# brontoguana/krasis

Measured on AMD Instinct MI355X. Metric: decode tok/s, Qwen3-Coder-Next Q4 @1 MI355X (KR_DECODE_FAST tolerance mode; both modes: value_exact / value_fast), higher is better.
Workload: dtype int4-g128 w x int16 act -> i32, f32 scales; 1 GPU; Qwen3-Coder-Next Q4 int4gpu on 1×MI355X (512-expert top-10, hybrid linear+GQA, FP8 KV); kv=FP8-E4M3 KV cache, kv_max_seq 256, layers=48, parallelism=one GPU holds the whole model (N > 1 lines: expert parallelism, see main_multi), hip_graph=True

## Files before the change

### krasis_amd/csrc/kr_decode.cpp

```cpp
#include <algorithm>
#include <hip/hip_runtime.h>

#include <cmath>
#include <cstring>
#include <memory>
#include <string>
#include <vector>

#include "../../include/krasis_hip.h"
#include "kr_decode_ops.h"
#include "kr_engine_internal.h"
#include "kr_kernels.h"
#include "kr_prefill.h"
#include "kr_router.h"
#include "kr_sampler.h"
#include <chrono>

#include "kr_decode_internal.h"
#include "kr_decode_fast.h"

static void prof_mark(kr_decode_store* s, int kind, hipStream_t st) {
    if (!s->prof) return;
    if (s->ev_used + 2 > s->ev_pool.size()) { for (int i = 0; i < 64; i++) { hipEvent_t e; (void)hipEventCreate(&e); s->ev_pool.push_back(e); } }
    if (kind >= 0) s->ev_kind.push_back(kind);
// ... 273 lines not shown
    for (auto& L : s->layers) if (L.mlp == MLP_MOE && L.moe_layer >= (int)eng->layers.size())
        return kr_fail(KR_ERR_VALUE, "moe_layer_idx %d out of range (engine has %zu MoE layers)", L.moe_layer, eng->layers.size());
    kr_engine_destroy(s->eng);
    s->eng = eng; s->own_eng = false; s->graph_ok = false; s->last_stream = nullptr;
    return KR_OK;
}

extern "C" int kr_decode_set_layer_moe(kr_decode_store* s, int layer, int moe_layer_idx, int shared_gate_up_wid, int shared_down_wid, int shared_gate_wid) {
    if (int rc = need_cfg(s)) return rc;
    if (layer < 0 || layer >= (int)s->layers.size()) return kr_fail(KR_ERR_VALUE, "layer %d out of range", layer);
    if (moe_layer_idx < 0 || (!s->own_eng && moe_layer_idx >= (int)s->eng->layers.size())) return kr_fail(KR_ERR_VALUE, "moe_layer_idx %d out of range", moe_layer_idx);
    if ((shared_gate_up_wid >= 0) != (shared_down_wid >= 0)) return kr_fail(KR_ERR_VALUE, "shared gate_up and down weights must be set together");
    for (int id : {shared_gate_up_wid, shared_down_wid, shared_gate_wid}) if (id >= 0) if (int rc = chk_wid(s, id, "set_decode_layer_moe")) return rc;
    DLayer& L = s->layers[layer];
    L.mlp = MLP_MOE; L.moe_layer = moe_layer_idx; L.sgu_wid = shared_gate_up_wid; L.sd_wid = shared_down_wid; L.sg_wid = shared_gate_wid;
    s->graph_ok = false;
    return KR_OK;
}

extern "C" int kr_decode_set_layer_dense(kr_decode_store* s, int layer, int gate_wid, int up_wid, int down_wid) {
    if (int rc = need_cfg(s)) return rc;
    if (layer < 0 || layer >= (int)s->layers.size()) return kr_fail(KR_ERR_VALUE, "layer %d out of range", layer);
    for (int id : {gate_wid, up_wid, down_wid}) if (int rc = chk_wid(s, id, "set_decode_layer_dense")) return rc;
    DLayer& L = s->layers[layer];
    L.mlp = MLP_DENSE; L.gate_wid = gate_wid; L.up_wid = up_wid; L.down_wid = down_wid;
    s->graph_ok = false;
    return KR_OK;
}

extern "C" int kr_decode_set_rope(kr_decode_store* s, const float* cos_t, const float* sin_t, int half_dim, int max_seq) {
    if (int rc = need_cfg(s)) return rc;
    KR_HIP(hipSetDevice(s->eng->device));
    if (int rc = upload_f32(s->rope_cos, cos_t, (size_t)half_dim * max_seq)) return rc;
    if (int rc = upload_f32(s->rope_sin, sin_t, (size_t)half_dim * max_seq)) return rc;
    s->rope_half = half_dim; s->max_rope_seq = max_seq; s->graph_ok = false;
    return KR_OK;
}

static size_t maxz(size_t a, size_t b) { return a > b ? a : b; }

extern "C" int kr_decode_finalize(kr_decode_store* s) {
    if (int rc = need_cfg(s)) return rc;
    if ((int)s->layers.size() != s->n_layers) return kr_fail(KR_ERR_STATE, "configured %d layers but %zu were added", s->n_layers, s->layers.size());
    KR_HIP(hipSetDevice(s->eng->device));
    size_t pa = 0, pb = 0, qb = 0, kb = 0, vb = 0, zb = 0, ro = 0, ao = 0, gb = 0, dg = 0, lb = 0, fq = 64;
    for (auto& L : s->layers) {
        if (L.attn == ATTN_LA) {
            pa = maxz(pa, s->weights[L.qkvz_wid]->rows); pb = maxz(pb, s->weights[L.ba_wid]->rows);
            qb = maxz(qb, (size_t)L.nv * L.dk); kb = maxz(kb, (size_t)L.nv * L.dk); vb = maxz(vb, (size_t)L.nv * L.dv); zb = maxz(zb, (size_t)L.nv * L.dv);
            ro = maxz(ro, (size_t)L.nv * L.dv); ao = maxz(ao, s->weights[L.out_wid]->cols); gb = maxz(gb, L.nv); fq = maxz(fq, (size_t)L.nk * 2 * L.dk);
        } else if (L.attn == ATTN_GQA) {
            pa = maxz(pa, s->weights[L.q_wid]->rows); kb = maxz(kb, s->weights[L.k_wid]->rows); vb = maxz(vb, s->weights[L.v_wid]->rows);
            qb = maxz(qb, (size_t)L.nh * L.hd); zb = maxz(zb, (size_t)L.nh * L.hd); ao = maxz(ao, s->weights[L.o_wid]->cols);
        }
        else if (L.attn == ATTN_MLA) {
            const size_t hd = (size_t)L.nd + L.rd;
            pa = maxz(pa, (size_t)L.nh * hd); kb = maxz(kb, (size_t)L.klr + L.rd); qb = maxz(qb, (size_t)L.nh * L.klr); zb = maxz(zb, (size_t)L.nh * L.rd);
            lb = maxz(lb, (size_t)L.nh * L.klr); ao = maxz(ao, maxz((size_t)L.nh * L.vhd, s->weights[L.o_wid]->cols));
            if (L.mq_wid < 0) pb = maxz(pb, maxz(s->weights[L.mqa_wid]->rows, s->weights[L.mqb_wid]->cols));
        }
        if (L.mlp == MLP_DENSE) dg = maxz(dg, 2 * (size_t)s->weights[L.down_wid]->cols);
    }
    ao = maxz(ao, (size_t)s->hidden);
    {
        const size_t kh = ((size_t)s->hidden + 127) / 128 * 128, ka = (ao + 127) / 128 * 128;
        if (s->img_in.ensure(kr_act_image_bytes((int)kh)) || s->img_post.ensure(kr_act_image_bytes((int)kh)) || s->img_post_bf16.ensure(kr_act_image_bytes((int)kh)) ||
            s->img_attn.ensure(kr_act_image_bytes((int)ka)))
            return kr_fail(KR_ERR_HIP, "hipMalloc of the activation images failed");
// ... 242 lines not shown
        a.q = (float*)s->f_qk.p;
        if (PROF_RC(PK_LA_RECUR, kr_launch_la_step_heads(a, (float*)L.recur_state.p, (const float*)L.la_norm_w.p, (float*)s->attn_out.p, s->eps, st, la_img)))
            return kr_fail(KR_ERR_VALUE, "unsupported linear-attention geometry");
    } else if (la_fused) {
        (void)PROF_RC(PK_LA_RECUR, kr_launch_la_step(a, (float*)L.recur_state.p, (const float*)L.la_norm_w.p, (float*)s->attn_out.p, s->eps, st, la_img));
    } else {
        PROF(PK_LA_CONV, kr_launch_la_conv(a, st));
        if (PROF_RC(PK_LA_RECUR, kr_launch_la_recurrent_gnorm((float*)L.recur_state.p, a.q, a.k, a.v, a.g, a.beta, a.z, (const float*)L.la_norm_w.p,
                                                             (float*)s->attn_out.p, L.nv, L.dk, L.dv, s->eps, st, la_img)))
            return kr_fail(KR_ERR_VALUE, "unsupported linear-attention geometry");
    }
    out_proj(cx, L.out_wid, o_img);
    return KR_OK;
}

static int attn_gqa(StepCtx& cx, DLayer& L, size_t li) {
    kr_decode_store* s = cx.s; hipStream_t st = cx.st;
    if (!L.kv_k.p) return kr_fail(KR_ERR_STATE, "set_decode_state was not called (no KV cache for layer %zu)", li);
    if (!cx.did_in) {
        const int wids[3] = {L.q_wid, L.k_wid, L.v_wid};
        float* ys[3] = {(float*)s->proj_a.p, (float*)s->kbuf.p, (float*)s->vbuf.p};
        proj_group(cx, wids, ys, 3, cx.in_img ? (const void*)s->img_in.p : (const void*)cx.hid, cx.in_img ? 2 : 1);
    }
    KrGqaArgs a{};
    a.step = (const KrStep*)s->step_dev.p; a.q_in = (const float*)s->proj_a.p; a.k_in = (const float*)s->kbuf.p; a.v_in = (const float*)s->vbuf.p;
    a.q_norm = L.q_norm_len ? (const float*)L.q_norm.p : nullptr; a.k_norm = L.k_norm_len ? (const float*)L.k_norm.p : nullptr;
    a.q_norm_per_head = L.q_norm_len == L.nh * L.hd; a.k_norm_per_head = L.k_norm_len == L.nkv * L.hd;
    a.rope_cos = (const float*)s->rope_cos.p; a.rope_sin = (const float*)s->rope_sin.p; a.rope_half = s->rope_half;
    a.k_cache = L.kv_k.p; a.v_cache = L.kv_v.p; a.kv_fp8 = s->kv_fp8; a.q_out = (float*)s->qbuf.p; a.gate = (float*)s->gatebuf.p;
    a.attn_out = (float*)s->attn_out.p; a.gated = L.gated; a.nh = L.nh; a.nkv = L.nkv; a.hd = L.hd; a.eps = s->eps; a.sm_scale = L.sm_scale;
    const bool o_img = cx.img_ok() && img_w(s, L.o_wid) && L.hd % 128 == 0 && s->weights[L.o_wid]->cols == L.nh * L.hd;
    a.img_out = o_img ? s->img_attn.p : nullptr;
    a.sc_g = s->kv_max_seq > s->gqa_split_min ? (float*)s->gqa_scores.p : nullptr;
    a.force_stream = s->opt_gqa_stream; a.tree_norm = cx.fast ? 1 : 0;
    if (s->attn_fast && a.sc_g) { a.fd_o = (float*)s->fd_o.p; a.fd_ml = (float*)s->fd_ml.p; }
    PROF(PK_GQA, { if (!(cx.fast && s->opt_gqa_fused && !a.sc_g && kr_launch_fgqa(a, s->kv_max_seq, st) == 0)) kr_launch_gqa(a, s->kv_max_seq, st); });
    out_proj(cx, L.o_wid, o_img);
    return KR_OK;
}

static void mla_lora_tail(StepCtx& cx, DLayer& L, float* q_full) {
    kr_decode_store* s = cx.s; hipStream_t st = cx.st;
    if (L.q_a_norm_len) PROF(PK_RMSNORM, kr_launch_rmsnorm_seq((float*)s->proj_b.p, (const float*)L.q_a_norm.p, s->weights[L.mqa_wid]->rows, s->eps, st));
    PROF(PK_MATVEC, kr_launch_matvec(mv(s, L.mqb_wid), s->proj_b.p, 1, q_full, st));
}

static int attn_mla(StepCtx& cx, DLayer& L, size_t li) {
    kr_decode_store* s = cx.s; hipStream_t st = cx.st;
    if (!L.kv_k.p) return kr_fail(KR_ERR_STATE, "set_decode_state was not called (no MLA cache for layer %zu)", li);
    if (L.mla_rope_seq < s->kv_max_seq) return kr_fail(KR_ERR_VALUE, "MLA rope table (%d) shorter than kv_max_seq (%d)", L.mla_rope_seq, s->kv_max_seq);
    float* kv_out = (float*)s->kbuf.p; float* q_full = (float*)s->proj_a.p;
    const bool lora = L.mq_wid < 0;
    if (!cx.did_in) {
        const int wids[2] = {L.kva_wid, lora ? L.mqa_wid : L.mq_wid};
        float* ys[2] = {kv_out, lora ? (float*)s->proj_b.p : q_full};
        proj_group(cx, wids, ys, 2, cx.hid, 1);
    }
    if (lora) mla_lora_tail(cx, L, q_full);
    KrMlaArgs a{};
    a.step = (const KrStep*)s->step_dev.p; a.kv_out = kv_out; a.q_full = q_full; a.kv_a_norm = (const float*)L.kv_a_norm.p; a.w_kc = (const float*)L.w_kc.p;
    a.w_vc = (const float*)L.w_vc.p; a.rope_cos = (const float*)L.mla_cos.p; a.rope_sin = (const float*)L.mla_sin.p;
    a.ckv_cache = L.kv_k.p; a.kpe_cache = L.kv_v.p; a.kv_fp8 = s->kv_fp8; a.q_abs = (float*)s->qbuf.p; a.q_pe = (float*)s->zbuf.p;
    a.attn_lat = (float*)s->latbuf.p; a.v_proj = (float*)s->attn_out.p;
    a.nh = L.nh; a.klr = L.klr; a.nd = L.nd; a.rd = L.rd; a.vhd = L.vhd; a.eps = s->eps; a.sm_scale = L.sm_scale;
    a.sc_g = s->kv_max_seq > s->mla_split_min ? (float*)s->gqa_scores.p : nullptr;
    if (s->attn_fast && a.sc_g) { a.fast = 1; a.fd_o = (float*)s->fd_o.p; a.fd_ml = (float*)s->fd_ml.p; }
    a.decode_fast = cx.fast ? 1 : 0; a.decode_fused = cx.fast && s->opt_gqa_fused ? 1 : 0;
// ... 264 lines not shown
        return KR_OK;
    }
    return enqueue_step(s, st);
}

extern "C" int kr_decode_set_kv_dtype(kr_decode_store* s, int kv_dtype) {
    if (int rc = chk_store(s)) return rc;
    if (kv_dtype != 0 && kv_dtype != 1) return kr_fail(KR_ERR_VALUE, "kv_dtype %d unknown (0 = FP16, 1 = FP8-E4M3)", kv_dtype);
    if (s->kv_fp8 != kv_dtype) for (auto& L : s->layers) if (L.attn == ATTN_GQA || L.attn == ATTN_MLA) { L.kv_k.release(); L.kv_v.release(); }
    s->kv_fp8 = kv_dtype; s->graph_ok = false;
    return KR_OK;
}

extern "C" int kr_decode_set_attention_mode(kr_decode_store* s, int mode) {
    if (int rc = chk_store(s)) return rc;
    if (mode < 0 || mode > 7) return kr_fail(KR_ERR_VALUE, "numerics mode %d unknown (bit 0 = KR_ATTN_FAST, bit 1 = KR_GEMM_FAST, bit 2 = KR_DECODE_FAST)", mode);
    s->attn_fast = mode & 1; s->gemm_fast = (mode >> 1) & 1; s->decode_fast = (mode >> 2) & 1; s->graph_ok = false;
    return KR_OK;
}

extern "C" int kr_decode_set_option(kr_decode_store* s, const char* name, int value) {
    if (int rc = chk_store(s)) return rc;
    if (!name) return kr_fail(KR_ERR_VALUE, "null option name");
    if (!strcmp(name, "gqa_stream")) { s->opt_gqa_stream = value != 0; s->graph_ok = false; return KR_OK; }
    if (!strcmp(name, "w2_combine")) { s->opt_w2_combine = value != 0; s->graph_ok = false; return KR_OK; }
    if (!strcmp(name, "la_heads")) { s->opt_la_heads = value != 0; s->graph_ok = false; return KR_OK; }
    if (!strcmp(name, "lm_fused")) { s->opt_lm_fused = value != 0; s->graph_ok = false; return KR_OK; }
    if (!strcmp(name, "gqa_fused")) { s->opt_gqa_fused = value != 0; s->graph_ok = false; return KR_OK; }
    if (!strcmp(name, "gemm_ring")) { kr_pfr_set_enabled(value); return KR_OK; }
    if (!strcmp(name, "la_conv_fused")) { s->opt_la_conv_fused = value != 0; return KR_OK; }
    if (!strcmp(name, "dense_fast")) { s->opt_dense_fast = value != 0; s->graph_ok = false; return KR_OK; }
    if (!strcmp(name, "slot_select")) { s->opt_slot_select = value != 0; s->graph_ok = false; return KR_OK; }
    if (!strcmp(name, "slot_rows_late_first")) { s->opt_slot_rows_late_first = value != 0; s->graph_ok = false; return KR_OK; }
    if (!strcmp(name, "norm_rows")) { s->opt_norm_rows = value != 0; return KR_OK; }
    if (!strcmp(name, "pfm_timing")) { s->opt_pfm_timing = value != 0; return KR_OK; }
    if (!strcmp(name, "generate_lookahead")) { s->opt_gen_lookahead = value != 0; return KR_OK; }
    if (!strcmp(name, "multi_sample_loop")) { s->opt_multi_sample_loop = value != 0; return KR_OK; }
    if (!strcmp(name, "multi_attn_fast")) { s->opt_multi_attn_fast = value != 0; return KR_OK; }
    if (!strcmp(name, "multi_attn_fast_paged")) { s->opt_multi_attn_fast_paged = value != 0; return KR_OK; }
    if (!strcmp(name, "multi_mla_fast")) { s->opt_multi_mla_fast = value != 0; return KR_OK; }
    if (!strcmp(name, "multi_extend_la_chunk")) { s->opt_multi_extend_la_chunk = value != 0; return KR_OK; }
    if (!strcmp(name, "multi_extend_exact_mfma")) { s->opt_multi_extend_exact_mfma = value != 0; return KR_OK; }
    if (!strcmp(name, "multi_extend_mla_exact_mfma")) { s->opt_multi_extend_mla_exact_mfma = value != 0; return KR_OK; }
    if (!strcmp(name, "multi_attn_exact_split")) { s->opt_multi_attn_exact_split = value != 0; return KR_OK; }
    if (!strcmp(name, "multi_attn_exact_split_min")) {
        if (value < 1) return kr_fail(KR_ERR_VALUE, "multi_attn_exact_split_min %d: at least 1", value);
        s->opt_multi_attn_exact_split_min = value; return KR_OK;
    }
    if (!strcmp(name, "multi_mla_exact_split")) { s->opt_multi_mla_exact_split = value != 0; return KR_OK; }
    if (!strcmp(name, "multi_extend_la_exact")) { s->opt_multi_extend_la_exact = value != 0; return KR_OK; }
    if (!strcmp(name, "multi_extend_la_exact_min")) {
        if (value < 2 || value > 1024) return kr_fail(KR_ERR_VALUE, "multi_extend_la_exact_min %d: must be in [2, 1024]", value);
        s->opt_multi_extend_la_exact_min = value; return KR_OK;
    }
    if (!strcmp(name, "multi_mla_exact_split_min")) {
        if (value < 1) return kr_fail(KR_ERR_VALUE, "multi_mla_exact_split_min %d: at least 1", value);
        s->opt_multi_mla_exact_split_min = value; return KR_OK;
    }
    if (!strcmp(name, "multi_extend_flash")) { s->opt_multi_extend_flash = value != 0; return KR_OK; }
    if (!strcmp(name, "multi_extend_mla_flash")) { s->opt_multi_extend_mla_flash = value != 0; return KR_OK; }
    if (!strcmp(name, "gguf_exact_pass")) { s->opt_gguf_exact_pass = value != 0; return KR_OK; }
    if (!strcmp(name, "gguf_exact_grouped")) { s->opt_gguf_exact_grouped = value != 0; return KR_OK; }
    if (!strcmp(name, "pass_few_rows")) { s->opt_pass_few_rows = value != 0; return KR_OK; }
    if (!strcmp(name, "pass_few_rows_max")) {
        if (value < 1 || value > 16) return kr_fail(KR_ERR_VALUE, "pass_few_rows_max %d: 1 .. 16", value);
        s->opt_pass_few_rows_max = value; return KR_OK;
// ... 238 lines not shown
```

### krasis_amd/csrc/kr_decode_fast.hip

```cpp
#include "kr_decode_fast.h"
#include "kr_gguf_dev.h"

#include "kr_device.h"
#include "kr_libm.h"
#include "kr_exact_dev.h"
#include "kr_matvec_dev.h"
#include "kr_topk.h"

typedef float f32x4 __attribute__((ext_vector_type(4)));
extern __shared__ __attribute__((aligned(16))) u32x4 kr_fsm[];

#ifdef KR_FTIMING
__device__ unsigned long long kr_fstamps[8][16];
#define KR_FSTAMP(k, i) do { if (blockIdx.x == gridDim.x / 2 && blockIdx.y == 0 && threadIdx.x == 0) kr_fstamps[k][i] = wall_clock64(); } while (0)
#define KR_FSTAMPY(k, i, row_) do { if (blockIdx.x == gridDim.x / 2 && (int)blockIdx.y == (row_) && threadIdx.x == 0) kr_fstamps[k][i] = wall_clock64(); } while (0)
extern "C" int kr_debug_fstamps(unsigned long long* out) { return (int)hipMemcpyFromSymbol(out, HIP_SYMBOL(kr_fstamps), sizeof(kr_fstamps)); }
__device__ unsigned long long kr_fwg[6][1024][3];
#define KR_FWG(k, i) do { if (threadIdx.x == 0) { const unsigned b_ = blockIdx.x + gridDim.x * blockIdx.y; if (b_ < 1024) { kr_fwg[k][b_][i] = wall_clock64(); \
        if ((i) == 0) kr_fwg[k][b_][2] = (unsigned long long)__builtin_amdgcn_s_getreg((4 << 0) | (0 << 6) | (31 << 11)) | ((unsigned long long)__builtin_amdgcn_s_getreg((20 << 0) | (0 << 6) | (3 << 11)) << 32); } } } while (0)
extern "C" int kr_debug_fwg(unsigned long long* out) { return (int)hipMemcpyFromSymbol(out, HIP_SYMBOL(kr_fwg), sizeof(kr_fwg)); }
#else
#define KR_FSTAMP(k, i) do { } while (0)
#define KR_FSTAMPY(k, i, y) do { } while (0)
#define KR_FWG(k, i) do { } while (0)
#endif

#define KR_FW2_LDS_MAX (64 * 1024)
#define KR_FU 16

__device__ __forceinline__ float kr_f_red8(float v) {
    v += __int_as_float(KR_DPP(__float_as_int(v), KR_DPP_XOR1));
    v += __int_as_float(KR_DPP(__float_as_int(v), KR_DPP_XOR2));
    v += __int_as_float(KR_DPP(__float_as_int(v), KR_DPP_HALF_MIRROR));
    return v;
}
__device__ __forceinline__ float kr_f_red16(float v) {
    v = kr_f_red8(v);
    v += __int_as_float(KR_DPP(__float_as_int(v), KR_DPP_MIRROR));
    return v;
}
__device__ __forceinline__ float kr_f_rl(float v, int l) { return __int_as_float(__builtin_amdgcn_readlane(__float_as_int(v), l)); }
__device__ __forceinline__ float kr_f_wave_sum(float v) {
    v = kr_f_red16(v);
    return (kr_f_rl(v, 0) + kr_f_rl(v, 16)) + (kr_f_rl(v, 32) + kr_f_rl(v, 48));
}
__device__ __forceinline__ float kr_f_wave_max(float v) {
    v = kr_red16_max_f32(v);
    return fmaxf(fmaxf(kr_f_rl(v, 0), kr_f_rl(v, 16)), fmaxf(kr_f_rl(v, 32), kr_f_rl(v, 48)));
}
__device__ __forceinline__ void kr_f_wave_sync() { __builtin_amdgcn_fence(__ATOMIC_ACQ_REL, "workgroup"); __builtin_amdgcn_wave_barrier(); }

template <int BITS, int NU, int FU = KR_FU> struct KrFw { u32x4 w[NU > 0 ? NU : FU]; uint32_t sc[NU > 0 ? NU : FU]; };

template <int BITS, int NU, int FU = KR_FU>
__device__ __forceinline__ void kr_f_fetch(KrFw<BITS, NU, FU>& p, const KrMatDev& m, const void* qbase, const uint32_t* sbase, int tile, int lane, int ub, int u1) {
    const int units = BITS == 4 ? m.ngp : m.ng;
    const u32x4* q = reinterpret_cast<const u32x4*>(qbase) + (size_t)tile * units * 64 + lane;
// ... 921 lines not shown

#define KR_FGQA_MAX 1024
template <int N, bool FP8> struct KrKvRaw { static constexpr int W = FP8 ? (N + 3) / 4 : (N + 1) / 2; uint32_t w[W]; };
template <int N, bool FP8>
__device__ __forceinline__ void kr_kv_raw_load(KrKvRaw<N, FP8>& r, const void* base, size_t elem) {
    constexpr int bytes = FP8 ? N : 2 * N;
    const char* p = reinterpret_cast<const char*>(base) + elem * (FP8 ? 1 : 2);
    if constexpr (bytes >= 16) {
#pragma unroll
        for (int i = 0; i < bytes / 16; i++) { const u32x4 v = *reinterpret_cast<const u32x4*>(p + 16 * i); r.w[4 * i] = v.x; r.w[4 * i + 1] = v.y; r.w[4 * i + 2] = v.z; r.w[4 * i + 3] = v.w; }
    } else if constexpr (bytes == 8) { const u32x2 v = *reinterpret_cast<const u32x2*>(p); r.w[0] = v.x; r.w[1] = v.y; }
    else if constexpr (bytes == 4) r.w[0] = *reinterpret_cast<const uint32_t*>(p);
    else if constexpr (bytes == 2) r.w[0] = *reinterpret_cast<const uint16_t*>(p);
    else r.w[0] = *reinterpret_cast<const uint8_t*>(p);
}
template <int N, bool FP8>
__device__ __forceinline__ void kr_kv_raw_f32(const KrKvRaw<N, FP8>& r, float (&x)[N]) {
#pragma unroll
    for (int i = 0; i < N; i++) {
        if constexpr (FP8) {
            const int w = (int)r.w[i >> 2];
            x[i] = (i & 3) == 0 ? __builtin_amdgcn_cvt_f32_fp8(w, 0) : ((i & 3) == 1 ? __builtin_amdgcn_cvt_f32_fp8(w, 1) : ((i & 3) == 2 ? __builtin_amdgcn_cvt_f32_fp8(w, 2) : __builtin_amdgcn_cvt_f32_fp8(w, 3)));
        } else {
            const uint16_t hb = (uint16_t)((i & 1) ? (r.w[i >> 1] >> 16) : (r.w[i >> 1] & 0xFFFFu));
            x[i] = (float)__builtin_bit_cast(_Float16, hb);
        }
    }
}
template <bool FP8> __device__ __forceinline__ float kr_kv_round(float v) {
    if constexpr (FP8) return kr_e4m3_to_f32(kr_f32_to_e4m3(v));
    else return (float)(_Float16)v;
}

template <int HD, bool FP8>
__global__ void __launch_bounds__(256) kr_fgqa_kernel(const KrStep* p_step, const float* p_q, const float* p_k, const float* p_v, const void* p_kc, const void* p_vc,
                                                      int p_nh, int p_nkv, const KrGqaArgs a) {
    constexpr int D16 = HD / 16;
    constexpr int DPL = HD / 64;
    constexpr int SB = 2;
    constexpr int PB = 8;
    __shared__ __attribute__((aligned(16))) float s_q[HD], s_k[HD], s_v[HD], s_sc[KR_FGQA_MAX + 64], s_part[4][HD];
    __shared__ float s_red[2][4];
    const int h = blockIdx.x, t = threadIdx.x, wave = t >> 6, lane = t & 63;
    const int grp = p_nh / p_nkv, kvh = h / grp;
    const int pos = p_step->pos, seq = pos + 1;
    const size_t rowe = (size_t)p_nkv * HD, headoff = (size_t)kvh * HD;
    const int d = t < HD ? t : HD - 1;
    const bool own = t < HD;
    const float qraw = a.gated ? p_q[(size_t)h * HD * 2 + d] : p_q[(size_t)h * HD + d];
    const float graw = a.gated ? p_q[(size_t)h * HD * 2 + HD + d] : 0.0f;
    const float kraw = p_k[headoff + d], vraw = p_v[headoff + d];
    const float qw = a.q_norm ? a.q_norm[(a.q_norm_per_head ? h * HD : 0) + d] : 1.0f;
    const float kw = a.k_norm ? a.k_norm[(a.k_norm_per_head ? kvh * HD : 0) + d] : 1.0f;
    const int d2 = a.rope_half;
    const bool rot = t < 2 * d2 && own;
    const int ri = rot ? (t < d2 ? t : t - d2) : 0;
    const float rc = a.rope_cos[(size_t)pos * d2 + ri], rs = a.rope_sin[(size_t)pos * d2 + ri];
    const int l16 = lane & 15, pw = lane >> 4;
    KrKvRaw<D16, FP8> kqA[SB], kqB[SB];
    auto issue_k = [&](KrKvRaw<D16, FP8> (&kq)[SB], int s0) {
#pragma unroll
        for (int u = 0; u < SB; u++) { const int sp = s0 + 16 * u + wave * 4 + pw; kr_kv_raw_load<D16, FP8>(kq[u], p_kc, (size_t)(sp < pos ? sp : 0) * rowe + headoff + l16 * D16); }
    };
    issue_k(kqA, 0);
    float sq = own ? qraw * qraw : 0.0f, sk = own ? kraw * kraw : 0.0f;
    sq = kr_f_wave_sum(sq); sk = kr_f_wave_sum(sk);
    if (lane == 0) { s_red[0][wave] = sq; s_red[1][wave] = sk; }
    __syncthreads();
    float qx = qraw, kx = kraw;
    if (a.q_norm) { const float ss = (s_red[0][0] + s_red[0][1]) + (s_red[0][2] + s_red[0][3]); qx = qraw * (kr_rms_inv(ss, HD, a.eps) * qw); }
    if (a.k_norm) { const float ss = (s_red[1][0] + s_red[1][1]) + (s_red[1][2] + s_red[1][3]); kx = kraw * (kr_rms_inv(ss, HD, a.eps) * kw); }
    if (own) { s_q[t] = qx; s_k[t] = kx; }
    __syncthreads();
    float qv = qx, kv = kx;
    if (rot) {
        if (t < d2) { qv = qx * rc - s_q[d2 + t] * rs; kv = kx * rc - s_k[d2 + t] * rs; }
        else { qv = qx * rc + s_q[t - d2] * rs; kv = kx * rc + s_k[t - d2] * rs; }
    }
    __syncthreads();
    if (own) {
        s_q[t] = qv; s_k[t] = kr_kv_round<FP8>(kv); s_v[t] = kr_kv_round<FP8>(vraw);
        if (h == kvh * grp) {
            const size_t o = (size_t)pos * rowe + headoff + t;
            kr_kv_store(const_cast<void*>(p_kc), o, kv, FP8 ? 1 : 0);
            kr_kv_store(const_cast<void*>(p_vc), o, vraw, FP8 ? 1 : 0);
        }
    }
    __syncthreads();
    float qreg[D16], knew[D16];
#pragma unroll
    for (int i = 0; i < D16; i++) { qreg[i] = s_q[l16 * D16 + i]; knew[i] = s_k[l16 * D16 + i]; }
    auto score_batch = [&](const KrKvRaw<D16, FP8> (&kq)[SB], int s0) {
#pragma unroll
        for (int u = 0; u < SB; u++) {
            const int sp = s0 + 16 * u + wave * 4 + pw;
            float kx_[D16];
            kr_kv_raw_f32<D16, FP8>(kq[u], kx_);
            float acc = 0.0f;
#pragma unroll
            for (int i = 0; i < D16; i++) acc = __builtin_fmaf(qreg[i], sp == pos ? knew[i] : kx_[i], acc);
            acc = kr_f_red16(acc);
            if (l16 == 0 && sp < seq) s_sc[sp] = acc * a.sm_scale;
        }
    };
    constexpr int SSTEP = 16 * SB;
    for (int s0 = 0; s0 < seq; s0 += 2 * SSTEP) {
        if (s0 + SSTEP < seq) issue_k(kqB, s0 + SSTEP);
        score_batch(kqA, s0);
        if (s0 + 2 * SSTEP < seq) issue_k(kqA, s0 + 2 * SSTEP);
        if (s0 + SSTEP < seq) score_batch(kqB, s0 + SSTEP);
    }
    KrKvRaw<DPL, FP8> vqA[PB], vqB[PB];
    auto issue_v = [&](KrKvRaw<DPL, FP8> (&vq)[PB], int s0) {
#pragma unroll
        for (int u = 0; u < PB; u++) { const int sp = s0 + 4 * u + wave; kr_kv_raw_load<DPL, FP8>(vq[u], p_vc, (size_t)(sp < pos ? sp : 0) * rowe + headoff + lane * DPL); }
    };
    issue_v(vqA, 0);
    __syncthreads();
    float mx = -__builtin_inff();
    for (int sp = t; sp < seq; sp += 256) mx = fmaxf(mx, s_sc[sp]);
    mx = kr_f_wave_max(mx);
    if (lane == 0) s_red[0][wave] = mx;
    __syncthreads();
    mx = fmaxf(fmaxf(s_red[0][0], s_red[0][1]), fmaxf(s_red[0][2], s_red[0][3]));
    float se = 0.0f;
    for (int sp = t; sp < seq; sp += 256) { const float e = kr_expf(s_sc[sp] - mx); s_sc[sp] = e; se += e; }
    se = kr_f_wave_sum(se);
    if (lane == 0) s_red[1][wave] = se;
    __syncthreads();
    const float inv = 1.0f / ((s_red[1][0] + s_red[1][1]) + (s_red[1][2] + s_red[1][3]));
    for (int sp = t; sp < seq; sp += 256) s_sc[sp] *= inv;
    float vnew[DPL];
#pragma unroll
    for (int i = 0; i < DPL; i++) vnew[i] = s_v[lane * DPL + i];
    __syncthreads();
    float o[DPL];
#pragma unroll
    for (int i = 0; i < DPL; i++) o[i] = 0.0f;
    auto pv_batch = [&](const KrKvRaw<DPL, FP8> (&vq)[PB], int s0) {
#pragma unroll
        for (int u = 0; u < PB; u++) {
            const int sp = s0 + 4 * u + wave;
            float vx[DPL];
            kr_kv_raw_f32<DPL, FP8>(vq[u], vx);
            const float pr = sp < seq ? s_sc[sp] : 0.0f;
#pragma unroll
            for (int i = 0; i < DPL; i++) o[i] = __builtin_fmaf(pr, sp == pos ? vnew[i] : vx[i], o[i]);
        }
    };
    constexpr int PSTEP = 4 * PB;
    for (int s0 = 0; s0 < seq; s0 += 2 * PSTEP) {
        if (s0 + PSTEP < seq) issue_v(vqB, s0 + PSTEP);
        pv_batch(vqA, s0);
        if (s0 + 2 * PSTEP < seq) issue_v(vqA, s0 + 2 * PSTEP);
        if (s0 + PSTEP < seq) pv_batch(vqB, s0 + PSTEP);
    }
#pragma unroll
    for (int i = 0; i < DPL; i++) s_part[wave][lane * DPL + i] = o[i];
    __syncthreads();
    float ov = 0.0f;
    if (own) {
        ov = (s_part[0][t] + s_part[1][t]) + (s_part[2][t] + s_part[3][t]);
        if (a.gated) ov *= 1.0f / (1.0f + kr_expf(-graw));
        a.attn_out[(size_t)h * HD + t] = ov;
        s_q[t] = ov;
    }
    if (a.img_out) {
        __syncthreads();
        const KrActLds Lg = kr_carve_lds(reinterpret_cast<u32x4*>(a.img_out), p_nh * HD, false);
        constexpr int nch = HD / 8;
        if (t < nch) {
            float v8[8];
            kr_load8(s_q, t, v8);
            float mxq = 0.0f;
#pragma unroll
            for (int i = 0; i < 8; i++) mxq = fmaxf(mxq, fabsf(v8[i]));
            float scale, invq;
            kr_group_scale(mxq, scale, invq);
            int q8[8];
            kr_quant8<false>(v8, invq, q8);
            const int gc = h * nch + t;
            kr_store_chunk<false>(Lg, gc, q8);
            if ((gc & 15) == 0) Lg.ascale[gc >> 4] = scale;
        }
    }
}

template <int KLR, int RD, bool FP8>
__global__ void __launch_bounds__(256) kr_fmla_kernel(const KrStep* p_step, const float* p_qabs, const float* p_qpe, const void* p_ckv, const void* p_kpe, float* p_out, float p_scale) {
    constexpr int DC = KLR / 16, DR = RD / 16, DPL = KLR / 64, SB = 2, PB = 8;
    __shared__ __attribute__((aligned(16))) float s_sc[KR_FGQA_MAX + 64], s_part[4][KLR];
    __shared__ float s_red[2][4];
    const int h = blockIdx.x, t = threadIdx.x, wave = t >> 6, lane = t & 63, l16 = lane & 15, pw = lane >> 4;
    const int pos = p_step->pos, seq = pos + 1;
    KrKvRaw<DC, FP8> kcA[SB], kcB[SB]; KrKvRaw<DR, FP8> krA[SB], krB[SB];
    auto issue_k = [&](KrKvRaw<DC, FP8> (&kc)[SB], KrKvRaw<DR, FP8> (&kr)[SB], int s0) {
#pragma unroll
        for (int u = 0; u < SB; u++) {
            const int sp = s0 + 16 * u + wave * 4 + pw, sr = sp < seq ? sp : 0;
            kr_kv_raw_load<DC, FP8>(kc[u], p_ckv, (size_t)sr * KLR + l16 * DC);
            kr_kv_raw_load<DR, FP8>(kr[u], p_kpe, (size_t)sr * RD + l16 * DR);
        }
    };
    float qc[DC], qr[DR];
#pragma unroll
    for (int i = 0; i < DC; i += 4) { const float4 v = *reinterpret_cast<const float4*>(p_qabs + (size_t)h * KLR + l16 * DC + i); qc[i] = v.x; qc[i + 1] = v.y; qc[i + 2] = v.z; qc[i + 3] = v.w; }
#pragma unroll
    for (int i = 0; i < DR; i += 4) { const float4 v = *reinterpret_cast<const float4*>(p_qpe + (size_t)h * RD + l16 * DR + i); qr[i] = v.x; qr[i + 1] = v.y; qr[i + 2] = v.z; qr[i + 3] = v.w; }
    issue_k(kcA, krA, 0);
    auto score_batch = [&](const KrKvRaw<DC, FP8> (&kc)[SB], const KrKvRaw<DR, FP8> (&kr)[SB], int s0) {
#pragma unroll
        for (int u = 0; u < SB; u++) {
            const int sp = s0 + 16 * u + wave * 4 + pw;
            float xc[DC], xr[DR];
            kr_kv_raw_f32<DC, FP8>(kc[u], xc); kr_kv_raw_f32<DR, FP8>(kr[u], xr);
            float acc = 0.0f, acr = 0.0f;
#pragma unroll
            for (int i = 0; i < DC; i++) acc = __builtin_fmaf(qc[i], xc[i], acc);
// ... 39 lines not shown
        for (int u = 0; u < PB; u++) {
            const int sp = s0 + 4 * u + wave;
            float vx[DPL];
            kr_kv_raw_f32<DPL, FP8>(vq[u], vx);
            const float pr = sp < seq ? s_sc[sp] : 0.0f;
#pragma unroll
            for (int i = 0; i < DPL; i++) o[i] = __builtin_fmaf(pr, vx[i], o[i]);
        }
    };
    constexpr int PSTEP = 4 * PB;
    for (int s0 = 0; s0 < seq; s0 += 2 * PSTEP) {
        if (s0 + PSTEP < seq) issue_v(vqB, s0 + PSTEP);
        pv_batch(vqA, s0);
        if (s0 + 2 * PSTEP < seq) issue_v(vqA, s0 + 2 * PSTEP);
        if (s0 + PSTEP < seq) pv_batch(vqB, s0 + PSTEP);
    }
#pragma unroll
    for (int i = 0; i < DPL; i++) s_part[wave][lane * DPL + i] = o[i];
    __syncthreads();
    for (int j = t; j < KLR; j += 256) p_out[(size_t)h * KLR + j] = (s_part[0][j] + s_part[1][j]) + (s_part[2][j] + s_part[3][j]);
}

int kr_launch_fmla(const KrMlaArgs& a, int max_seq, hipStream_t st) {
    if (!a.step || max_seq > KR_FGQA_MAX || a.sc_g || a.rd != 64 || (a.klr != 512 && a.klr != 256)) return 1;
#define KR_FMLA(K_, F_) hipLaunchKernelGGL((kr_fmla_kernel<K_, 64, F_>), dim3(a.nh), dim3(256), 0, st, a.step, (const float*)a.q_abs, (const float*)a.q_pe, (const void*)a.ckv_cache, (const void*)a.kpe_cache, a.attn_lat, a.sm_scale)
    if (a.klr == 512) { if (a.kv_fp8) KR_FMLA(512, true); else KR_FMLA(512, false); }
    else { if (a.kv_fp8) KR_FMLA(256, true); else KR_FMLA(256, false); }
#undef KR_FMLA
    return 0;
}

int kr_launch_fgqa(const KrGqaArgs& a, int max_seq, hipStream_t st) {
    if (max_seq > KR_FGQA_MAX || a.sc_g || a.nh % a.nkv || 2 * a.rope_half > a.hd || (a.img_out && a.hd % 128)) return 1;
#define KR_FGQA(H_, F_) hipLaunchKernelGGL((kr_fgqa_kernel<H_, F_>), dim3(a.nh), dim3(256), 0, st, a.step, a.q_in, a.k_in, a.v_in, (const void*)a.k_cache, (const void*)a.v_cache, a.nh, a.nkv, a)
    if (a.hd == 256) { if (a.kv_fp8) KR_FGQA(256, true); else KR_FGQA(256, false); }
    else if (a.hd == 128) { if (a.kv_fp8) KR_FGQA(128, true); else KR_FGQA(128, false); }
    else if (a.hd == 64) { if (a.kv_fp8) KR_FGQA(64, true); else KR_FGQA(64, false); }
    else return 1;
#undef KR_FGQA
    return 0;
}

template <int BITS, int KS, int MODE>
static int kr_fdm_launch_nu2(const KrFdmArgs& a, int nu, dim3 grid, size_t lds, hipStream_t st) {
    const void* p0 = MODE == 0 ? a.img : ((MODE == 1 && a.emb) ? nullptr : (const void*)a.hid_in);
    const float* p1 = (MODE == 1 && !a.first) ? a.res_in : nullptr;
    const int Kp = a.mm.m[0].ng * 128;
#define KR_FDM(N_) hipLaunchKernelGGL((kr_fdm_kernel<BITS, KS, N_, MODE>), grid, dim3(256), lds, st, p0, p1, a.norm_w, Kp, a)
    switch (nu) {
        case 2: KR_FDM(2); break;
        case 4: KR_FDM(4); break;
        case 8: KR_FDM(8); break;
        case 16: KR_FDM(16); break;
        default: KR_FDM(0); break;
    }
#undef KR_FDM
    return 0;
}
template <int BITS, int KS>
static int kr_fdm_launch_nu(const KrFdmArgs& a, int nu, dim3 grid, size_t lds, hipStream_t st) {
    if (a.mode == 0) return kr_fdm_launch_nu2<BITS, KS, 0>(a, nu, grid, lds, st);
    if (a.mode == 2) return kr_fdm_launch_nu2<BITS, KS, 2>(a, nu, grid, lds, st);
    return kr_fdm_launch_nu2<BITS, KS, 1>(a, nu, grid, lds, st);
}

int kr_launch_fdm(const KrFdmArgs& a, hipStream_t st) {
    const KrMatDev& m0 = a.mm.m[0];
    const int bits = m0.bits, K = m0.ng * 128;
    for (int i = 1; i < a.mm.n; i++) if (a.mm.m[i].bits != bits || a.mm.m[i].ng != m0.ng) return 1;
    if ((a.mode == 1 || a.mode == 2) && (K > 4096 || K != m0.K)) return 1;
    if (a.conv_state && (a.conv_mi < 0 || a.conv_mi >= a.mm.n || a.mm.m[a.conv_mi].N != a.nk * (2 * a.dk + 2 * a.hr * a.dv) || a.gate_mi < 0 || a.gate_mi >= a.mm.n ||
                         a.mm.m[a.gate_mi].N != a.nk * 2 * a.hr || !a.ge_out || !a.beta_out)) return 1;
// ... 132 lines not shown
```

### krasis_amd/csrc/kr_decode_internal.h

```cpp
#pragma once
#include <hip/hip_runtime.h>

#include <memory>
#include <vector>

#include "kr_decode_ops.h"
#include "kr_engine_internal.h"
#include "kr_multi.h"
#include "kr_page_pool.h"
#include "kr_spec.h"

struct DWeight { MatSet ms; int rows = 0, cols = 0; };

enum { ATTN_NONE = 0, ATTN_LA = 1, ATTN_GQA = 2, ATTN_MLA = 3 };
enum { MLP_NONE = 0, MLP_MOE = 1, MLP_DENSE = 2 };

struct DLayer {
    int input_norm = -1, post_norm = -1;
    int attn = ATTN_NONE, mlp = MLP_NONE;
    int qkvz_wid = -1, ba_wid = -1, out_wid = -1, nk = 0, nv = 0, dk = 0, dv = 0, kd = 4; float la_scale = 1.0f;
    DevBuf conv_w, a_log, dt_bias, la_norm_w, conv_state, recur_state;
    int q_wid = -1, k_wid = -1, v_wid = -1, o_wid = -1, gated = 0, nh = 0, nkv = 0, hd = 0; float sm_scale = 1.0f;
    DevBuf q_norm, k_norm, kv_k, kv_v; int q_norm_len = 0, k_norm_len = 0;
    int kva_wid = -1, mq_wid = -1, mqa_wid = -1, mqb_wid = -1, klr = 0, nd = 0, rd = 0, vhd = 0, q_a_norm_len = 0;
// ... 16 lines not shown
    DevBuf lc_scratch;
    DevBuf xm_rows;
    bool mla_fd_ready = false;
    struct Sampler { float temperature = 0.0f, top_p = 1.0f, penalty = 0.0f; int top_k = 0; };
    std::vector<Sampler> smp; size_t smp_words = 0;
    DevBuf smp_seen, smp_rng;
    DevBuf smp_rows, smp_work, smp_sorted, smp_keys, smp_temp, smp_probs; size_t smp_temp_bytes = 0;
    DevBuf smp_hyp;
    DevBuf v_rec, v_tab, v_out, v_keep; std::vector<KrMultiLaCommit> v_host; std::vector<int> v_la_of;
    bool v_pending = false, v_sampled = false, v_has64 = false, v_has128 = false; int v_nv_max = 0, v_dv_max = 0; size_t v_rows = 0;
    std::vector<int32_t> v_match; hipStream_t v_st = nullptr;
    hipEvent_t ev = nullptr;
    DevBuf sw_stage, sw_pools, sw_pieces; void* sw_pinned = nullptr; size_t sw_half = 0; hipStream_t sw_stream = nullptr; hipEvent_t sw_ev[4] = {nullptr, nullptr, nullptr, nullptr};
    ~kr_multi_state() {
        if (ev) (void)hipEventDestroy(ev);
        for (hipEvent_t e : sw_ev) if (e) (void)hipEventDestroy(e);
        if (sw_stream) (void)hipStreamDestroy(sw_stream);
        if (sw_pinned) (void)hipHostFree(sw_pinned);
    }
};

struct kr_standalone_state;
struct kr_decode_store {
    kr_standalone_state* standalone = nullptr;
    kr_engine* eng = nullptr; int device = 0; bool own_eng = false;
    int group_size = 128; bool norm_bias_one = false;
    std::vector<std::unique_ptr<DWeight>> weights;
    std::vector<std::unique_ptr<DevBuf>> norms; std::vector<int> norm_len;
    bool configured = false;
    int hidden = 0, n_layers = 0, vocab = 0, topk = 0, scoring = 1, norm_topk = 1, final_norm = -1, lm_head = -1;
    float eps = 1e-6f, rsf = 1.0f;
    DevBuf embedding;
    std::vector<DLayer> layers;
    DevBuf rope_cos, rope_sin; int rope_half = 0, max_rope_seq = 0;
    int kv_max_seq = 0;
    DevBuf hid, res, proj_a, proj_b, qbuf, kbuf, vbuf, zbuf, gbuf, betabuf, gatebuf, latbuf, recur_out, attn_out, logits, gate_val, tok;
    DevBuf dense_gu;
    DevBuf hid2, res2, r_counter, argmax_scratch;
    int kv_fp8 = 0;
    DevBuf img_in, img_post, img_post_bf16, img_attn;
    int opt_gqa_stream = 0, opt_pfm_timing = 0, opt_norm_rows = 1, opt_la_conv_fused = 1, opt_gqa_fused = 1, opt_lm_fused = 1, opt_la_heads = 1, opt_w2_combine = 1, opt_dense_fast = 1, opt_slot_select = 1, opt_slot_rows_late_first = 1;
    int opt_multi_sample_loop = 0;
    int opt_gguf_exact_pass = 0;
    int opt_gguf_exact_grouped = 1;
    int opt_multi_attn_fast_paged = 0;
    int opt_multi_attn_fast = 0;
    int opt_multi_mla_fast = 0;
    int opt_multi_extend_flash = 0;
    int opt_multi_extend_la_chunk = 0;
    int opt_multi_attn_exact_split = 0;
    int opt_multi_attn_exact_split_min = 512;
    int opt_multi_extend_la_exact = 0;
    int opt_multi_extend_la_exact_min = 8;
    int opt_multi_mla_exact_split = 0;
    int opt_multi_mla_exact_split_min = 512;
    int opt_multi_extend_exact_mfma = 0;
    int opt_multi_extend_mla_exact_mfma = 0;
    int opt_multi_extend_mla_flash = 0;
    int opt_pass_few_rows = 0;
    int opt_pass_few_rows_max = 16;
    int opt_pass_few_rows_group = 0;
    int opt_slot_swap_chunk_bytes = KR_SLOT_CHUNK_DEFAULT;
    int64_t path_counts[KR_MPC_COUNT] = {};
    int opt_gen_lookahead = 0;
    int opt_ep_graph = 0;
    uint64_t ep_generation_seen = 0;
    int ep_eager_steps = 0;
    int* gen_ring = nullptr; int gen_ring_n = 0; hipEvent_t gen_ev[2] = {nullptr, nullptr};
    int decode_fast = 0; DevBuf f_qk;
    int gemm_fast = 0;
    int attn_fast = 0; DevBuf fd_o, fd_ml;
    DevBuf gqa_scores; int gqa_split_min = 1024, mla_split_min = 512;
    DevBuf smp_seen, smp_keys, smp_temp, smp_probs, smp_rng; size_t smp_temp_bytes = 0;
    DevBuf pf_scores;
// ... 36 lines not shown
```

### krasis_amd/csrc/kr_decode_ops.h

```cpp
#pragma once
#include <hip/hip_runtime.h>
#include <stdint.h>

struct KrStep { int token; int pos; };

struct KrLaArgs {
    const float* qkvz; const float* ba; float* conv_state; const float* conv_w; const float* a_log; const float* dt_bias;
    float scale; float *q, *k, *v, *z, *g, *beta; int nk, nv, dk, dv, hr;
};
struct KrGqaArgs {
    const KrStep* step;
    const float *q_in, *k_in, *v_in;
    const float *q_norm, *k_norm; int q_norm_per_head, k_norm_per_head;
    const float *rope_cos, *rope_sin; int rope_half;
    void *k_cache, *v_cache; int kv_fp8;
    float *q_out, *gate, *attn_out;
    int gated, nh, nkv, hd; float eps, sm_scale;
    void* img_out;
    float* sc_g;
    float *fd_o, *fd_ml;
    int tree_norm;
    int force_stream;
};

struct KrFdFlashArgs {
    const KrStep* step; const float* q;
    const void *k_cache, *v_cache;
    float *fd_o, *fd_ml;
    int nh, nkv; float sm_scale;
    const float* gate; int gated; float* out; void* img_out;
};
int kr_fd_flash_chunk(int max_seq);
size_t kr_fd_flash_chunks(int max_seq);
int kr_fd_flash_prepare(int hd, int fp8);
int kr_launch_fd_flash(const KrFdFlashArgs& a, int hd, int fp8, int max_seq, hipStream_t st);
int kr_gqa_attn_prepare(int max_seq, int hd, int fp8);

struct KrMlaArgs {
    const KrStep* step;
    const float* kv_out;
    const float* q_full;
    const float *kv_a_norm, *w_kc, *w_vc, *rope_cos, *rope_sin;
    void *ckv_cache, *kpe_cache;
    int kv_fp8;
    float* sc_g;
    float *fd_o, *fd_ml; int fast;
    float *q_abs, *q_pe, *attn_lat, *v_proj;
    int nh, klr, nd, rd, vhd; float eps, sm_scale;
    int pos0; int ld_kv, ld_q;
    int decode_fast;
    int decode_fused;
    int absorb_done;
    float* pf_sc; int pf_sc_ld;
};
void kr_launch_mla(const KrMlaArgs& a, int max_seq, hipStream_t s, int n_tok = 1);
// ... 27 lines not shown
```

Before: 642.5 tok/s.

## Prefetch a window of KV cache rows before norm/rope in fused GQA decode kernel

Adds a templated prefetch path to the fused GQA decode kernel. It issues K loads for the first 128 positions into registers and V rows into registers (later staged into LDS) at kernel start, before the q/k norm and rope work. The aim is to hide the KV cache memory latency behind that prologue instead of serialising it. The path is on by default through a new attn_prefetch option, and in exchange it raises register and shared memory pressure, which may reduce occupancy. Timing stamps are also extended for KR_FTIMING builds.

```diff
diff --git a/krasis_amd/csrc/kr_decode.cpp b/krasis_amd/csrc/kr_decode.cpp
--- a/krasis_amd/csrc/kr_decode.cpp
+++ b/krasis_amd/csrc/kr_decode.cpp
@@ -329,8 +329,7 @@
     if (int rc = need_cfg(s)) return rc;
     KR_HIP(hipSetDevice(s->eng->device));
     if (int rc = upload_f32(s->rope_cos, cos_t, (size_t)half_dim * max_seq)) return rc;
-    if (int rc = upload_f32(s->rope_sin, sin_t, (size_t)half_dim * max_seq)) return rc;
-    s->rope_half = half_dim; s->max_rope_seq = max_seq; s->graph_ok = false;
+    if (int rc = upload_f32(s->rope_sin, sin_t, (size_t)half_dim * max_seq)) return rc;    s->rope_half = half_dim; s->max_rope_seq = max_seq; s->graph_ok = false;
     return KR_OK;
 }
 
@@ -639,7 +638,7 @@
     const bool o_img = cx.img_ok() && img_w(s, L.o_wid) && L.hd % 128 == 0 && s->weights[L.o_wid]->cols == L.nh * L.hd;
     a.img_out = o_img ? s->img_attn.p : nullptr;
     a.sc_g = s->kv_max_seq > s->gqa_split_min ? (float*)s->gqa_scores.p : nullptr;
-    a.force_stream = s->opt_gqa_stream; a.tree_norm = cx.fast ? 1 : 0;
+    a.force_stream = s->opt_gqa_stream; a.tree_norm = cx.fast ? 1 : 0; a.attn_prefetch = s->opt_attn_prefetch;
     if (s->attn_fast && a.sc_g) { a.fd_o = (float*)s->fd_o.p; a.fd_ml = (float*)s->fd_ml.p; }
     PROF(PK_GQA, { if (!(cx.fast && s->opt_gqa_fused && !a.sc_g && kr_launch_fgqa(a, s->kv_max_seq, st) == 0)) kr_launch_gqa(a, s->kv_max_seq, st); });
     out_proj(cx, L.o_wid, o_img);
@@ -970,6 +969,7 @@
     if (!strcmp(name, "dense_fast")) { s->opt_dense_fast = value != 0; s->graph_ok = false; return KR_OK; }
     if (!strcmp(name, "slot_select")) { s->opt_slot_select = value != 0; s->graph_ok = false; return KR_OK; }
     if (!strcmp(name, "slot_rows_late_first")) { s->opt_slot_rows_late_first = value != 0; s->graph_ok = false; return KR_OK; }
+    if (!strcmp(name, "attn_prefetch")) { s->opt_attn_prefetch = value != 0; s->graph_ok = false; return KR_OK; }
     if (!strcmp(name, "norm_rows")) { s->opt_norm_rows = value != 0; return KR_OK; }
     if (!strcmp(name, "pfm_timing")) { s->opt_pfm_timing = value != 0; return KR_OK; }
     if (!strcmp(name, "generate_lookahead")) { s->opt_gen_lookahead = value != 0; return KR_OK; }
diff --git a/krasis_amd/csrc/kr_decode_fast.hip b/krasis_amd/csrc/kr_decode_fast.hip
--- a/krasis_amd/csrc/kr_decode_fast.hip
+++ b/krasis_amd/csrc/kr_decode_fast.hip
@@ -11,7 +11,9 @@
 extern __shared__ __attribute__((aligned(16))) u32x4 kr_fsm[];
 
 #ifdef KR_FTIMING
-__device__ unsigned long long kr_fstamps[8][16];
+__device__ unsigned long long kr_fstamps[10][16];
+#define KR_FDEP_S(x) asm volatile("" :: "s"(x))
+#define KR_FDEP_V(x) asm volatile("" :: "v"(x))
 #define KR_FSTAMP(k, i) do { if (blockIdx.x == gridDim.x / 2 && blockIdx.y == 0 && threadIdx.x == 0) kr_fstamps[k][i] = wall_clock64(); } while (0)
 #define KR_FSTAMPY(k, i, row_) do { if (blockIdx.x == gridDim.x / 2 && (int)blockIdx.y == (row_) && threadIdx.x == 0) kr_fstamps[k][i] = wall_clock64(); } while (0)
 extern "C" int kr_debug_fstamps(unsigned long long* out) { return (int)hipMemcpyFromSymbol(out, HIP_SYMBOL(kr_fstamps), sizeof(kr_fstamps)); }
@@ -23,6 +25,8 @@
 #define KR_FSTAMP(k, i) do { } while (0)
 #define KR_FSTAMPY(k, i, y) do { } while (0)
 #define KR_FWG(k, i) do { } while (0)
+#define KR_FDEP_S(x) do { } while (0)
+#define KR_FDEP_V(x) do { } while (0)
 #endif
 
 #define KR_FW2_LDS_MAX (64 * 1024)
@@ -1010,18 +1014,29 @@
     else return (float)(_Float16)v;
 }
 
-template <int HD, bool FP8>
+#define KR_FGQA_WIN 128
+template <int HD, bool FP8, bool PF>
 __global__ void __launch_bounds__(256) kr_fgqa_kernel(const KrStep* p_step, const float* p_q, const float* p_k, const float* p_v, const void* p_kc, const void* p_vc,
                                                       int p_nh, int p_nkv, const KrGqaArgs a) {
     constexpr int D16 = HD / 16;
     constexpr int DPL = HD / 64;
     constexpr int SB = 2;
     constexpr int PB = 8;
+    constexpr int SSTEP = 16 * SB, PSTEP = 4 * PB;
+    constexpr int RB = HD * (FP8 ? 1 : 2);
+    constexpr int W0 = PF ? KR_FGQA_WIN : 0, NKB = W0 / SSTEP;
+    constexpr int WV = PF ? (KR_FGQA_WIN * RB <= 32768 ? KR_FGQA_WIN : 32768 / RB) : 0, NVB = WV / PSTEP;
+    constexpr int VR = RB / 16, NVC = WV * VR / 256;
     __shared__ __attribute__((aligned(16))) float s_q[HD], s_k[HD], s_v[HD], s_sc[KR_FGQA_MAX + 64], s_part[4][HD];
+    __shared__ __attribute__((aligned(16))) uint32_t s_vw[PF ? WV * RB / 4 : 4];
     __shared__ float s_red[2][4];
+    KR_FSTAMP(8, 0);
     const int h = blockIdx.x, t = threadIdx.x, wave = t >> 6, lane = t & 63;
     const int grp = p_nh / p_nkv, kvh = h / grp;
     const int pos = p_step->pos, seq = pos + 1;
+    if constexpr (PF)
+        asm volatile("" :: "s"(pos), "s"(a.gated), "s"(a.q_norm), "s"(a.k_norm), "s"(a.q_norm_per_head), "s"(a.k_norm_per_head), "s"(a.rope_half), "s"(a.rope_cos),
+                     "s"(a.rope_sin), "s"(a.eps), "s"(a.sm_scale), "s"(a.attn_out), "s"(a.img_out));
     const size_t rowe = (size_t)p_nkv * HD, headoff = (size_t)kvh * HD;
     const int d = t < HD ? t : HD - 1;
     const bool own = t < HD;
@@ -1033,14 +1048,34 @@
     const int d2 = a.rope_half;
     const bool rot = t < 2 * d2 && own;
     const int ri = rot ? (t < d2 ? t : t - d2) : 0;
+    KR_FDEP_S(pos); KR_FSTAMP(8, 1);
     const float rc = a.rope_cos[(size_t)pos * d2 + ri], rs = a.rope_sin[(size_t)pos * d2 + ri];
     const int l16 = lane & 15, pw = lane >> 4;
     KrKvRaw<D16, FP8> kqA[SB], kqB[SB];
+    KrKvRaw<DPL, FP8> vqA[PB], vqB[PB];
+    KrKvRaw<D16, FP8> kwin[PF ? NKB : 1][SB];
+    u32x4 vwin[PF ? NVC : 1];
     auto issue_k = [&](KrKvRaw<D16, FP8> (&kq)[SB], int s0) {
 #pragma unroll
         for (int u = 0; u < SB; u++) { const int sp = s0 + 16 * u + wave * 4 + pw; kr_kv_raw_load<D16, FP8>(kq[u], p_kc, (size_t)(sp < pos ? sp : 0) * rowe + headoff + l16 * D16); }
     };
-    issue_k(kqA, 0);
+    auto issue_v = [&](KrKvRaw<DPL, FP8> (&vq)[PB], int s0) {
+#pragma unroll
+        for (int u = 0; u < PB; u++) { const int sp = s0 + 4 * u + wave; kr_kv_raw_load<DPL, FP8>(vq[u], p_vc, (size_t)(sp < pos ? sp : 0) * rowe + headoff + lane * DPL); }
+    };
+    if constexpr (PF) {
+#pragma unroll
+        for (int b = 0; b < NKB; b++) issue_k(kwin[b], b * SSTEP);
+#pragma unroll
+        for (int i = 0; i < NVC; i++) {
+            const int c = t + 256 * i, sp = c / VR;
+            vwin[i] = *reinterpret_cast<const u32x4*>(reinterpret_cast<const char*>(p_vc) + ((size_t)(sp < pos ? sp : 0) * rowe + headoff) * (FP8 ? 1 : 2) + (c % VR) * 16);
+        }
+        if (W0 < seq) issue_k(kqA, W0);
+        if (WV < seq) issue_v(vqA, WV);
+        KR_FSTAMP(8, 12);
+    } else issue_k(kqA, 0);
+    KR_FDEP_V(qraw); KR_FDEP_V(kraw); KR_FDEP_V(vraw); KR_FSTAMP(8, 2);
     float sq = own ? qraw * qraw : 0.0f, sk = own ? kraw * kraw : 0.0f;
     sq = kr_f_wave_sum(sq); sk = kr_f_wave_sum(sk);
     if (lane == 0) { s_red[0][wave] = sq; s_red[1][wave] = sk; }
@@ -1065,6 +1100,7 @@
         }
     }
     __syncthreads();
+    KR_FSTAMP(8, 3);
     float qreg[D16], knew[D16];
 #pragma unroll
     for (int i = 0; i < D16; i++) { qreg[i] = s_q[l16 * D16 + i]; knew[i] = s_k[l16 * D16 + i]; }
@@ -1081,19 +1117,22 @@
             if (l16 == 0 && sp < seq) s_sc[sp] = acc * a.sm_scale;
         }
     };
-    constexpr int SSTEP = 16 * SB;
-    for (int s0 = 0; s0 < seq; s0 += 2 * SSTEP) {
+    if constexpr (PF) {
+#pragma unroll
+        for (int b = 0; b < NKB; b++)
+            if (b * SSTEP < seq) { score_batch(kwin[b], b * SSTEP); KR_FSTAMP(8, 4 + b); }
+    }
+    for (int s0 = W0; s0 < seq; s0 += 2 * SSTEP) {
         if (s0 + SSTEP < seq) issue_k(kqB, s0 + SSTEP);
-        score_batch(kqA, s0);
+        score_batch(kqA, s0); KR_FSTAMP(8, 4 + ((s0 / SSTEP) & 7));
         if (s0 + 2 * SSTEP < seq) issue_k(kqA, s0 + 2 * SSTEP);
-        if (s0 + SSTEP < seq) score_batch(kqB, s0 + SSTEP);
-    }
-    KrKvRaw<DPL, FP8> vqA[PB], vqB[PB];
-    auto issue_v = [&](KrKvRaw<DPL, FP8> (&vq)[PB], int s0) {
-#pragma unroll
-        for (int u = 0; u < PB; u++) { const int sp = s0 + 4 * u + wave; kr_kv_raw_load<DPL, FP8>(vq[u], p_vc, (size_t)(sp < pos ? sp : 0) * rowe + headoff + lane * DPL); }
-    };
-    issue_v(vqA, 0);
+        if (s0 + SSTEP < seq) { score_batch(kqB, s0 + SSTEP); KR_FSTAMP(8, 4 + ((s0 / SSTEP + 1) & 7)); }
+    }
+    if constexpr (!PF) issue_v(vqA, 0);
+    else {
+#pragma unroll
+        for (int i = 0; i < NVC; i++) reinterpret_cast<u32x4*>(s_vw)[t + 256 * i] = vwin[i];
+    }
     __syncthreads();
     float mx = -__builtin_inff();
     for (int sp = t; sp < seq; sp += 256) mx = fmaxf(mx, s_sc[sp]);
@@ -1112,6 +1151,7 @@
 #pragma unroll
     for (int i = 0; i < DPL; i++) vnew[i] = s_v[lane * DPL + i];
     __syncthreads();
+    KR_FSTAMP(9, 0);
     float o[DPL];
 #pragma unroll
     for (int i = 0; i < DPL; i++) o[i] = 0.0f;
@@ -1123,15 +1163,24 @@
             kr_kv_raw_f32<DPL, FP8>(vq[u], vx);
             const float pr = sp < seq ? s_sc[sp] : 0.0f;
 #pragma unroll
-            for (int i = 0; i < DPL; i++) o[i] = __builtin_fmaf(pr, sp == pos ? vnew[i] : vx[i], o[i]);
+            for (int i = 0; i < DPL; i++) o[i] = __builtin_fmaf(pr, sp < pos ? vx[i] : (sp == pos ? vnew[i] : 0.0f), o[i]);
         }
     };
-    constexpr int PSTEP = 4 * PB;
-    for (int s0 = 0; s0 < seq; s0 += 2 * PSTEP) {
+    if constexpr (PF) {
+#pragma unroll
+        for (int b = 0; b < NVB; b++)
+            if (b * PSTEP < seq) {
+                KrKvRaw<DPL, FP8> vq[PB];
+#pragma unroll
+                for (int u = 0; u < PB; u++) kr_kv_raw_load<DPL, FP8>(vq[u], s_vw, (size_t)(b * PSTEP + 4 * u + wave) * HD + lane * DPL);
+                pv_batch(vq, b * PSTEP); KR_FSTAMP(9, 1 + b);
+            }
+    }
+    for (int s0 = WV; s0 < seq; s0 += 2 * PSTEP) {
         if (s0 + PSTEP < seq) issue_v(vqB, s0 + PSTEP);
-        pv_batch(vqA, s0);
+        pv_batch(vqA, s0); KR_FSTAMP(9, 1 + ((s0 / PSTEP) & 7));
         if (s0 + 2 * PSTEP < seq) issue_v(vqA, s0 + 2 * PSTEP);
-        if (s0 + PSTEP < seq) pv_batch(vqB, s0 + PSTEP);
+        if (s0 + PSTEP < seq) { pv_batch(vqB, s0 + PSTEP); KR_FSTAMP(9, 1 + ((s0 / PSTEP + 1) & 7)); }
     }
 #pragma unroll
     for (int i = 0; i < DPL; i++) s_part[wave][lane * DPL + i] = o[i];
@@ -1162,6 +1211,7 @@
             if ((gc & 15) == 0) Lg.ascale[gc >> 4] = scale;
         }
     }
+    KR_FSTAMP(9, 9);
 }
 
 template <int KLR, int RD, bool FP8>
@@ -1267,12 +1317,14 @@
 
 int kr_launch_fgqa(const KrGqaArgs& a, int max_seq, hipStream_t st) {
     if (max_seq > KR_FGQA_MAX || a.sc_g || a.nh % a.nkv || 2 * a.rope_half > a.hd || (a.img_out && a.hd % 128)) return 1;
-#define KR_FGQA(H_, F_) hipLaunchKernelGGL((kr_fgqa_kernel<H_, F_>), dim3(a.nh), dim3(256), 0, st, a.step, a.q_in, a.k_in, a.v_in, (const void*)a.k_cache, (const void*)a.v_cache, a.nh, a.nkv, a)
+#define KR_FGQA_PF(H_, F_, P_) hipLaunchKernelGGL((kr_fgqa_kernel<H_, F_, P_>), dim3(a.nh), dim3(256), 0, st, a.step, a.q_in, a.k_in, a.v_in, (const void*)a.k_cache, (const void*)a.v_cache, a.nh, a.nkv, a)
+#define KR_FGQA(H_, F_) do { if (a.attn_prefetch) KR_FGQA_PF(H_, F_, true); else KR_FGQA_PF(H_, F_, false); } while (0)
     if (a.hd == 256) { if (a.kv_fp8) KR_FGQA(256, true); else KR_FGQA(256, false); }
     else if (a.hd == 128) { if (a.kv_fp8) KR_FGQA(128, true); else KR_FGQA(128, false); }
     else if (a.hd == 64) { if (a.kv_fp8) KR_FGQA(64, true); else KR_FGQA(64, false); }
     else return 1;
 #undef KR_FGQA
+#undef KR_FGQA_PF
     return 0;
 }
 
diff --git a/krasis_amd/csrc/kr_decode_internal.h b/krasis_amd/csrc/kr_decode_internal.h
--- a/krasis_amd/csrc/kr_decode_internal.h
+++ b/krasis_amd/csrc/kr_decode_internal.h
@@ -72,14 +72,13 @@
     float eps = 1e-6f, rsf = 1.0f;
     DevBuf embedding;
     std::vector<DLayer> layers;
-    DevBuf rope_cos, rope_sin; int rope_half = 0, max_rope_seq = 0;
-    int kv_max_seq = 0;
+    DevBuf rope_cos, rope_sin; int rope_half = 0, max_rope_seq = 0;    int kv_max_seq = 0;
     DevBuf hid, res, proj_a, proj_b, qbuf, kbuf, vbuf, zbuf, gbuf, betabuf, gatebuf, latbuf, recur_out, attn_out, logits, gate_val, tok;
     DevBuf dense_gu;
     DevBuf hid2, res2, r_counter, argmax_scratch;
     int kv_fp8 = 0;
     DevBuf img_in, img_post, img_post_bf16, img_attn;
-    int opt_gqa_stream = 0, opt_pfm_timing = 0, opt_norm_rows = 1, opt_la_conv_fused = 1, opt_gqa_fused = 1, opt_lm_fused = 1, opt_la_heads = 1, opt_w2_combine = 1, opt_dense_fast = 1, opt_slot_select = 1, opt_slot_rows_late_first = 1;
+    int opt_gqa_stream = 0, opt_pfm_timing = 0, opt_norm_rows = 1, opt_la_conv_fused = 1, opt_gqa_fused = 1, opt_lm_fused = 1, opt_la_heads = 1, opt_w2_combine = 1, opt_dense_fast = 1, opt_slot_select = 1, opt_slot_rows_late_first = 1, opt_attn_prefetch = 1;
     int opt_multi_sample_loop = 0;
     int opt_gguf_exact_pass = 0;
     int opt_gguf_exact_grouped = 1;
diff --git a/krasis_amd/csrc/kr_decode_ops.h b/krasis_amd/csrc/kr_decode_ops.h
--- a/krasis_amd/csrc/kr_decode_ops.h
+++ b/krasis_amd/csrc/kr_decode_ops.h
@@ -21,6 +21,7 @@
     float *fd_o, *fd_ml;
     int tree_norm;
     int force_stream;
+    int attn_prefetch;
 };
 
 struct KrFdFlashArgs {
```

After: 647.8 tok/s, median of 6. Within noise of the previous version (+0.8%).
